# terran-project/terran

Measured on AMD Instinct MI355X. Metric: frames/sec 1080p detect+embed+pose, higher is better.
Workload: dtype f16x3: operands x = hi + lo (two IEEE halfs, 22 bits), 3 f16 MFMAs per product, f32 accumulate; float32-grade results; 1 GPU; BASELINE configs[4]: 1080p detect+embed+pose; Detection(short_side=416) + Recognition(top-2) + Estimation(short_side=184); 32 frames per GPU per step resident in HBM; random-init weights; precision=f16x3, frames_per_gpu_step=32, faces_per_frame=2, resident_batch_reused=True, batches_in_flight_per_gpu=2

## Files before the change

include/terran_amd.h:

```cpp
#ifndef TERRAN_AMD_H
#define TERRAN_AMD_H

#include <stddef.h>
#include <stdint.h>

#ifdef __cplusplus
extern "C" {
#endif

#define TA_OK 0
#define TA_E_INVALID (-1)
#define TA_E_DEVICE (-2)
#define TA_E_CAPACITY (-3)
#define TA_E_OVERFLOW (-4)
#define TA_E_RANGE (-5)

#define TA_MODEL_RETINAFACE 1
#define TA_MODEL_ARCFACE 2
#define TA_MODEL_OPENPOSE 3

typedef struct ta_ctx ta_ctx;
typedef struct ta_model ta_model;
typedef struct ta_frames ta_frames;

// ... 109 lines not shown
int ta_jpeg_encode_last_opt_stats(const ta_ctx* ctx, double* ms);

int ta_model_load(ta_ctx* ctx, int kind, const void* blob, size_t bytes, ta_model** out);
int ta_program_check(int kind, const void* blob, size_t bytes, char* msg, size_t msg_capacity);
void ta_model_free(ta_model* m);
int ta_model_kind(const ta_model* m);

int ta_model_forward_frames(ta_model* m, const ta_frames* frames);
int ta_model_forward_crops(ta_model* m, const uint8_t* crops_nchw_bgr, int n);
int ta_model_tensor_shape(ta_model* m, int tensor, int* n, int* c, int* h, int* w);
int ta_model_read_tensor(ta_model* m, int tensor, int ch_off, int ch, float* dst_nchw);

int ta_model_tensor_unscale(const ta_model* m, int tensor, float* out, int capacity);
int ta_model_debug_amax(ta_model* m, int enable, float* out, int capacity);
int ta_model_graph_probe(ta_model* m, int reps, double* out_ms);

int ta_retinaface_run(ta_model* m, const ta_frames* frames, float score_thr, float nms_thr,
                      int capacity, int32_t* counts, float* boxes, float* landmarks, float* scores,
                      int32_t* required);
int ta_retinaface_postprocess(ta_ctx* ctx, const float* const heads[9], int n, int h, int w,
                              float score_thr, float nms_thr, int capacity, int32_t* counts,
                              float* boxes, float* landmarks, float* scores, int32_t* required);

int ta_arcface_embed_crops(ta_model* m, const uint8_t* crops_nchw_bgr, int n, int normalize, float* out);
int ta_arcface_embed_faces(ta_model* m, const ta_frames* frames, const int32_t* frame_index,
                           const double* inv_affine, int n, int normalize, float* out,
                           uint8_t* crops_out);
int ta_arcface_embed_faces_multi(ta_model* m, const ta_frames* const* frames, int n_sources, const int32_t* source_index,
                                 const int32_t* frame_index, const double* inv_affine, int n, int normalize,
                                 float* out, uint8_t* crops_out);
int ta_cosine_distance(ta_ctx* ctx, const float* a, int na, const float* b, int nb, int dim, float* out);

int ta_openpose_run(ta_model* m, const ta_frames* frames, double scale, int capacity,
                    int32_t* counts, int32_t* keypoints, double* scores, int32_t* required);
int ta_openpose_group(ta_ctx* ctx, const float* pafs, const float* heatmaps, int n, int h, int w,
                      double scale, int capacity, int32_t* counts, int32_t* keypoints,
                      double* scores, int32_t* required);
int ta_openpose_last_stats(const ta_ctx* ctx, int64_t* peaks, int64_t* connections);

int ta_openpose_debug_read(ta_ctx* ctx, int n, int cap_peaks, int32_t* peak_counts, int32_t* peaks_yx,
                           float* peak_scores, int cap_conn, int32_t* conn_counts, int32_t* conn_ij,
                           float* conn_scores);

int ta_bicubic_x8(ta_ctx* ctx, const float* maps, int n, int c, int h, int w, float* out);

#define TA_CONV_AUTO 0
// ... 22 lines not shown
```

terran_amd/csrc/conv_dwpw.hip:

```cpp
#include <stdlib.h>

#include "conv_common.h"

TA_TRACE_READER(ta_debug_trace_read_dwpw)

template <int WAVES_M, int WAVES_N, int WM_TILES, int WN_TILES, int PREC = PREC_F32>
__global__ __launch_bounds__(256, 2) void conv_dwpw(const ta_conv_launch p) {
  constexpr int BN = WAVES_M * WM_TILES * 32;
  constexpr int BM = WAVES_N * WN_TILES * 32;
  constexpr int QA = BN / 32;
  constexpr int RP = BM / 32;
  constexpr int STAGE = (BN + BM) * 32;
  static_assert(WAVES_M * WAVES_N == 4, "4 waves per workgroup");
  extern __shared__ __attribute__((aligned(16))) float lds[];

  const int tid = threadIdx.x;
  const int lane = tid & 63;
  const int wave = __builtin_amdgcn_readfirstlane(tid >> 6);
  const int wm = wave / WAVES_N;
  const int wn = wave % WAVES_N;
  const int n_ct = p.coutp / BN;
  const int bid = blockIdx.x;
  const int grp = bid >> 3, xcd = bid & 7;
  const int ct = grp % n_ct;
// ... 84 lines not shown
  const int b_row0 = BN + wn * WN_TILES * 32 + frow;

  const int S = p.n_slabs;
  if (wave == 0) TA_STAMP(17);
  produce(0, 0);
  if (wave == 0) TA_STAMP(18);
  for (int s = 0; s < S; ++s) {
    asm volatile("s_waitcnt vmcnt(0)" ::: "memory");
    __syncthreads();
    if (s == 0 && wave == 0) TA_STAMP(19);
    if (s + 1 < S) produce(s + 1, (s + 1) & 1);
    const float* st = lds + (s & 1) * STAGE;
    conv_slab_mma<WM_TILES, WN_TILES, PREC>(st, acc, a_row0, b_row0, fsw, fcb, lane);
  }
  if (wave == 0) TA_STAMP(20);
  if constexpr (PREC != PREC_F32) {
    if (dw_amax > TA_F16_MAX_BITS) *p.range_flag = 1;
    if (p.amax_index >= 0 && dw_amax) atomicMax((unsigned*)p.range_flag + TA_AMAX_SLOT0 + 2 * p.amax_index + 1, dw_amax);
  }
  conv_finish_sym<WAVES_M, WAVES_N, WM_TILES, WN_TILES>(p, acc, lds, ct0, pt0, wm, wn, tid, lane, HoWo);
  if (wave == 0) TA_STAMP(23);
}

template <int WAVES_M, int WAVES_N, int WM_TILES, int WN_TILES>
__global__ __launch_bounds__(256, 2) void rf_dwpw_kernel(const ta_conv_launch p) {
  constexpr int BN = WAVES_M * WM_TILES * 32, BM = WAVES_N * WN_TILES * 32;
  constexpr int QA = BN / 32, RP = BM / 32, STAGE = (BN + BM) * 32;
  static_assert(WAVES_M * WAVES_N == 4 && (RP == 2 || RP == 4), "4 waves; 64 or 128 pixels per tile");
  extern __shared__ __attribute__((aligned(16))) float lds[];
  const int tid = threadIdx.x;
  const int lane = tid & 63;
  const int wave = __builtin_amdgcn_readfirstlane(tid >> 6);
  const int wm = wave / WAVES_N, wn = wave % WAVES_N;
  const int n_ct = p.coutp / BN;
  const int bid = blockIdx.x;
  const int grp = bid >> 3, xcd = bid & 7;
  const int ct = grp % n_ct;
  const int n_pt = (p.M + BM - 1) / BM;
  const int pt = ta_xcd_tile(n_pt, xcd, grp / n_ct);
  if (pt < 0) return;
  const int ct0 = ct * BN, pt0 = pt * BM;
  const int HoWo = p.Ho * p.Wo;
  const int C = p.dw_c, S = p.n_slabs;

  f32x4 pre[4];
  {
    const int pco = ct0 + 8 * (tid % (BN / 8));
// ... 29 lines not shown
      const int t = q * 4 + wave;
      __builtin_amdgcn_global_load_lds(GLB_PTR(a_src[q] + (size_t)s * a_slab_bytes), LDS_PTR(base + t * 256), 16, 0, 0);
    }
  };

  const int c4 = tid & 7;
  const __amdgpu_buffer_rsrc_t rsrc = __builtin_amdgcn_make_buffer_rsrc((void*)p.in, 0, -1, 0x00020000);
  int voff[RP];
#pragma unroll
  for (int j = 0; j < RP; ++j) {
    const int row = (tid >> 3) + 32 * j;
    int pix = pt0 + row;
    if (pix >= p.M) pix = 0;
    const int img = pix / HoWo;
    const int rem = pix - img * HoWo;
    const int y = rem / p.Wo;
    const int x = rem - y * p.Wo;
    voff[j] = 4 * (img * p.in_img + y * p.dw_stride * p.in_row + x * p.dw_stride * p.in_pix + p.in_off0) + 16 * c4;
  }
  const int row_b = 4 * p.in_row, pix_b = 4 * p.in_pix;

  unsigned dw_amax = 0;
  typedef unsigned u32x4 __attribute__((ext_vector_type(4)));
  auto produce = [&](int s, int stage) {
    float* base = lds + stage * STAGE;
    const int ch = s * 32 + c4 * 4;
    f32x4 w9[9], bias;
#pragma unroll
    for (int t = 0; t < 9; ++t) w9[t] = *(const f32x4*)(wl + t * C + ch);
    bias = *(const f32x4*)(wl + 9 * C + ch);
#pragma unroll
    for (int j0 = 0; j0 < RP; j0 += 2) {
      f32x4 v[2][9];
#pragma unroll
      for (int jj = 0; jj < 2; ++jj)
#pragma unroll
        for (int ky = 0; ky < 3; ++ky)
#pragma unroll
          for (int kx = 0; kx < 3; ++kx)
            v[jj][ky * 3 + kx] = __builtin_bit_cast(f32x4, (u32x4)__builtin_amdgcn_raw_buffer_load_b128(rsrc, voff[j0 + jj], ky * row_b + kx * pix_b + s * 128, 0));
#pragma unroll
      for (int jj = 0; jj < 2; ++jj) {
        const int row = (tid >> 3) + 32 * (j0 + jj);
        f32x4 acc = bias;
#pragma unroll
        for (int t = 0; t < 9; ++t)
#pragma unroll
          for (int e = 0; e < 4; ++e) acc[e] = __builtin_fmaf(v[jj][t][e], w9[t][e], acc[e]);
#pragma unroll
        for (int e = 0; e < 4; ++e) acc[e] = ta_relu(acc[e]);
        dw_amax = ta_amax4(dw_amax, acc);
        unsigned h0, h1, l0, l1;
        ta_pack2<true>(acc[0], acc[1], h0, l0);
        ta_pack2<true>(acc[2], acc[3], h1, l1);
        const int sw = (row >> 1) & 7;
        float* r = base + (BN + row) * 32 + (c4 & 1) * 2;
        *(uint2*)(r + (((c4 >> 1)) ^ sw) * 4) = make_uint2(h0, h1);
        *(uint2*)(r + ((4 + (c4 >> 1)) ^ sw) * 4) = make_uint2(l0, l1);
      }
    }
  };

  f32x16 acc[WM_TILES][WN_TILES];
// ... 19 lines not shown
        al[a] = *(const bf16x8*)(st + (a_row0 + a * 32) * 32 + ((4 + 2 * kg + t) ^ fsw) * 4);
      }
#pragma unroll
      for (int b = 0; b < WN_TILES; ++b) {
        bh[b] = *(const bf16x8*)(st + (b_row0 + b * 32) * 32 + ((2 * kg + t) ^ fsw) * 4);
        bl[b] = *(const bf16x8*)(st + (b_row0 + b * 32) * 32 + ((4 + 2 * kg + t) ^ fsw) * 4);
      }
#pragma unroll
      for (int a = 0; a < WM_TILES; ++a)
#pragma unroll
        for (int b = 0; b < WN_TILES; ++b) acc[a][b] = ta_mfma16<PREC_F16X3>(al[a], bh[b], acc[a][b]);
#pragma unroll
      for (int a = 0; a < WM_TILES; ++a)
#pragma unroll
        for (int b = 0; b < WN_TILES; ++b) acc[a][b] = ta_mfma16<PREC_F16X3>(ah[a], bl[b], acc[a][b]);
#pragma unroll
      for (int a = 0; a < WM_TILES; ++a)
#pragma unroll
        for (int b = 0; b < WN_TILES; ++b) acc[a][b] = ta_mfma16<PREC_F16X3>(ah[a], bh[b], acc[a][b]);
    }
  };

  dma_w(0, 0);
#pragma unroll
  for (int i = 0; i < WG; ++i)
    if (tid + 256 * i < n_gran) *(f32x4*)(wl + (tid + 256 * i) * 4) = wtmp[i];
  for (int g = tid + 256 * WG; g < n_gran; g += 256)
    *(f32x4*)(wl + g * 4) = g * 4 < 9 * C ? *(const f32x4*)(p.dw_w + g * 4) : *(const f32x4*)(p.dw_bias + (g * 4 - 9 * C));
  __syncthreads();
  produce(0, 0);
  for (int s = 0; s < S; ++s) {
    asm volatile("s_waitcnt vmcnt(0) lgkmcnt(0)" ::: "memory");
    __syncthreads();
    if (s + 1 < S) {
      dma_w(s + 1, (s + 1) & 1);
      produce(s + 1, (s + 1) & 1);
    }
    mma(s);
  }
  if (dw_amax > TA_F16_MAX_BITS) *p.range_flag = 1;
  if (p.amax_index >= 0 && dw_amax) atomicMax((unsigned*)p.range_flag + TA_AMAX_SLOT0 + 2 * p.amax_index + 1, dw_amax);

  constexpr int NCH = BN / 4, G = BN / 8, RPI = 256 / G;
  __syncthreads();
#pragma unroll
  for (int b = 0; b < WN_TILES; ++b) {
    const int row = (wn * WN_TILES + b) * 32 + (lane & 31);
#pragma unroll
    for (int a = 0; a < WM_TILES; ++a)
#pragma unroll
      for (int j = 0; j < 4; ++j) {
        const int c = ((wm * WM_TILES + a) * 32 + 8 * j + 4 * (lane >> 5)) >> 2;
        *(f32x4*)(lds + (row * NCH + (c ^ (row & (NCH - 1)))) * 4) =
            f32x4{acc[a][b][4 * j], acc[a][b][4 * j + 1], acc[a][b][4 * j + 2], acc[a][b][4 * j + 3]};
      }
  }
  __syncthreads();
  const int k8 = tid % G, r0 = tid / G;
  const int co = ct0 + 8 * k8;
// ... 24 lines not shown
        ta_split_store8<1>(o, v, am);
        amax = max(amax, am);
      } else {
        *(f32x4*)o = *(const f32x4*)v;
        *(f32x4*)(o + 16) = *(const f32x4*)(v + 4);
        if (chk) {
#pragma unroll
          for (int e = 0; e < 8; ++e) amax = max(amax, ta_absbits(v[e]));
        }
      }
      x += RPI;
      while (x >= p.Wo) {
        x -= p.Wo;
        if (++y == p.Ho) {
          y = 0;
          ++img;
        }
      }
    }
  }
  ta_range_report(p, amax);
}

template <int WAVES_M, int WAVES_N, int WM_TILES, int WN_TILES>
static int launch_rf_dwpw(ta_ctx* ctx, const ta_conv_launch& p) {
  constexpr int BN = WAVES_M * WM_TILES * 32, BM = WAVES_N * WN_TILES * 32;
  const int groups = ta_tile_grid(p, BN, BM).groups;
  const size_t lds_bytes = 2 * (size_t)(BN + BM) * 32 * sizeof(float) + (size_t)40 * p.dw_c;
  auto kern = rf_dwpw_kernel<WAVES_M, WAVES_N, WM_TILES, WN_TILES>;
  TA_NOTE_KERNEL(ctx, "rf_dwpw_kernel<%d,%d,%d,%d>", WAVES_M, WAVES_N, WM_TILES, WN_TILES);
  TA_SET_LDS_ATTR(ctx, kern, lds_bytes);
  hipLaunchKernelGGL(kern, dim3(groups * 8), dim3(256), lds_bytes, ctx->stream, p);
  TA_HIP(ctx, hipGetLastError());
  return TA_OK;
}

template <int WAVES_M, int WAVES_N, int WM_TILES, int WN_TILES, int PREC>
static int launch_dwpw_cfg(ta_ctx* ctx, const ta_conv_launch& p) {
  constexpr int BN = WAVES_M * WM_TILES * 32;
  constexpr int BM = WAVES_N * WN_TILES * 32;
  const int groups = ta_tile_grid(p, BN, BM).groups;
  const size_t lds_bytes = 2 * (size_t)(BN + BM) * 32 * sizeof(float);
  auto kern = conv_dwpw<WAVES_M, WAVES_N, WM_TILES, WN_TILES, PREC>;
  TA_NOTE_KERNEL(ctx, "conv_dwpw<%d,%d,%d,%d,%d>", WAVES_M, WAVES_N, WM_TILES, WN_TILES, PREC);
  TA_SET_LDS_ATTR(ctx, kern, lds_bytes);
  hipLaunchKernelGGL(kern, dim3(groups * 8), dim3(256), lds_bytes, ctx->stream, p);
  TA_HIP(ctx, hipGetLastError());
  return TA_OK;
}

int ta_launch_dwpw(ta_ctx* ctx, const ta_conv_launch& p_in, double flops) {
  if (p_in.M <= 0) return TA_OK;
  ta_conv_launch p = p_in;
  p.range_flag = ctx->range_flag;
  if ((p.prec != PREC_F32 && p.prec != PREC_F16X3) || p.in_fmt != TA_FMT_F32 || p.coutp % 32 || p.cout % 4 || (p.out_ch & 7) || p.dw_c % 4 || !p.dw_w ||
      !p.dw_bias || p.n_slabs * 32 < p.dw_c)
    return ta_fail(ctx, TA_E_INVALID, "dw+pw: needs the f32 or f16x3 mode, float32 input activations and 4-aligned channels");
  ta_prof_scope scope(ctx, 0, flops);
  ctx->cur_flops = flops;
#ifdef TA_CONV_TRACE
  p.trace_block = ctx->conv_trace_block;
#endif
  if (p.prec == PREC_F16X3) {
    const bool generic_only = getenv("TA_DWPW_GENERIC") != nullptr;
    const bool lean_ok = !generic_only && p.dw_c % 32 == 0 && p.dw_c == p.n_slabs * 32 && p.dw_c <= 1024 && p.cout % 8 == 0 && p.act == TA_ACT_RELU &&
                         (p.out_fmt == TA_FMT_F32 || p.out_fmt == TA_FMT_SPLIT16);
    if (lean_ok) {
      if (p.coutp % 128 == 0) return launch_rf_dwpw<2, 2, 2, 1>(ctx, p);
      if (p.coutp % 64 == 0) return launch_rf_dwpw<2, 2, 1, 1>(ctx, p);
      return launch_rf_dwpw<1, 4, 1, 1>(ctx, p);
    }
    if (p.coutp % 128 == 0) return launch_dwpw_cfg<2, 2, 2, 2, PREC_F16X3>(ctx, p);
    if (p.coutp % 64 == 0) return launch_dwpw_cfg<1, 4, 2, 1, PREC_F16X3>(ctx, p);
    return launch_dwpw_cfg<1, 4, 1, 1, PREC_F16X3>(ctx, p);
  }
  if (p.coutp % 128 == 0) return launch_dwpw_cfg<2, 2, 2, 2, PREC_F32>(ctx, p);
  if (p.coutp % 64 == 0) return launch_dwpw_cfg<1, 4, 2, 1, PREC_F32>(ctx, p);
  return launch_dwpw_cfg<1, 4, 1, 1, PREC_F32>(ctx, p);
}
```

terran_amd/csrc/retinaface_post.hip:

```cpp
#include <string.h>
#include <vector>

#include "act_format.h"
#include "ta_internal.h"

typedef float f32x4 __attribute__((ext_vector_type(4)));
#define RF_THREADS 1024
#define RF_LDS_KEYS 8192
#define RF_FAST_C 1024
#define RF_FAST_LDS (24 * 1024 + (RF_FAST_C / 64) * (RF_FAST_C / 64 + 1) / 2 * 64 * 8)
#define RF_LDS_MAX (159 * 1024)

struct rf_level {
  const float* head;
  int img, row, pix, off0;
  int fh, fw, stride;
  int t0;
  float ref[2][4];
};

struct rf_params {
  rf_level lv[3];
  int T;
  int cls_is_prob;
  float score_thr, nms_thr;
  float margin;
  unsigned long long* keys;
  int p_max;
  float* boxes;
  float* lmks;
  float* scores;
  int* keep;
  int* counts;
  int* ncand;
  long long* dbg;
  int fast_max;
};

__device__ __forceinline__ const float* rf_cell(const rf_level& L, int img, int t, int& a) {
  const int cell = t >> 1;
  a = t & 1;
  const int y = cell / L.fw, x = cell - y * L.fw;
  return L.head + (size_t)img * L.img + (size_t)y * L.row + (size_t)x * L.pix + L.off0;
}

__device__ __forceinline__ float rf_score(const rf_params& p, int img, int t) {
  const int l = t >= p.lv[2].t0 ? 2 : (t >= p.lv[1].t0 ? 1 : 0);
  int a;
  const float* c = rf_cell(p.lv[l], img, t - p.lv[l].t0, a);
  if (p.cls_is_prob) return c[2 + a];
  const float bg = c[a], fg = c[2 + a];
  const float m = fmaxf(bg, fg);
  const float eb = expf(bg - m), ef = expf(fg - m);
  return ef / (eb + ef);
}

__device__ __forceinline__ unsigned long long rf_readlane64(unsigned long long v, int l) {
  const unsigned lo = (unsigned)__builtin_amdgcn_readlane((int)(unsigned)v, l);
  const unsigned hi = (unsigned)__builtin_amdgcn_readlane((int)(unsigned)(v >> 32), l);
  return ((unsigned long long)hi << 32) | lo;
}

__device__ __forceinline__ int rf_row_off(int i, int W) {
  const int b = i >> 6;
  return 64 * (b * W - b * (b - 1) / 2) + (i - 64 * b) * (W - b);
}

__global__ __launch_bounds__(RF_THREADS) void rf_select_kernel(const rf_params p) {
  extern __shared__ __attribute__((aligned(16))) unsigned char smem[];
  unsigned long long* lkeys = (unsigned long long*)smem;
  unsigned* flags = (unsigned*)(smem + (size_t)RF_LDS_KEYS * 8);
  int* wave_tot = (int*)(flags + ((p.T + 31) / 32 + 3) / 4 * 4);
  int& s_base = wave_tot[16];

  const int img = blockIdx.x;
  const int tid = threadIdx.x, lane = tid & 63, wv = tid >> 6;
  unsigned long long* gkeys = p.keys + (size_t)img * p.p_max;

  if (p.dbg && tid == 0) p.dbg[img * 8 + 0] = wall_clock64();
  const int ncell = p.T >> 1;
  const int perc = (ncell + RF_THREADS - 1) / RF_THREADS;
  const int c0 = tid * perc, c1 = (c0 + perc < ncell) ? c0 + perc : ncell;
  const int per = 2 * perc, a0 = 2 * c0, a1 = 2 * c1;
  int cnt = 0;
  unsigned long long bits = 0;
  if (c0 < c1) {
    int l = a0 >= p.lv[2].t0 ? 2 : (a0 >= p.lv[1].t0 ? 1 : 0);
    const int cell = (a0 - p.lv[l].t0) >> 1;
    int y = cell / p.lv[l].fw, x = cell - y * p.lv[l].fw;
    const float* c = p.lv[l].head + (size_t)img * p.lv[l].img + (size_t)y * p.lv[l].row + (size_t)x * p.lv[l].pix + p.lv[l].off0;
    for (int q = c0; q < c1; q += 4) {
      f32x4 v[4];
#pragma unroll
      for (int k = 0; k < 4; ++k) {
        v[k] = *(const f32x4*)c;
        if (q + k + 1 < c1) {
          c += p.lv[l].pix;
          if (++x == p.lv[l].fw) {
            x = 0;
            ++y;
            c = p.lv[l].head + (size_t)img * p.lv[l].img + (size_t)y * p.lv[l].row + p.lv[l].off0;
          }
          if (l < 2 && 2 * (q + k + 1) == p.lv[l + 1].t0) {
            ++l;
            x = y = 0;
            c = p.lv[l].head + (size_t)img * p.lv[l].img + p.lv[l].off0;
          }
        }
// ... 3 lines not shown
#pragma unroll
        for (int a = 0; a < 2; ++a) {
          if (q + k >= c1) continue;
          bool pass;
          if (p.cls_is_prob) {
            pass = v[k][2 + a] >= p.score_thr;
          } else {
            const float bg = v[k][a], fg = v[k][2 + a];
            pass = false;
            if (!(fg - bg < p.margin)) {
              const float m = fmaxf(bg, fg);
              const float eb = expf(bg - m), ef = expf(fg - m);
              pass = ef / (eb + ef) >= p.score_thr;
            }
          }
          if (pass) {
            ++cnt;
            const int o = 2 * (q + k - c0) + a;
            if (o < 64) bits |= 1ull << o;
          }
        }
    }
  }
  int incl = cnt;
#pragma unroll
  for (int d = 1; d < 64; d <<= 1) {
    const int o = __shfl_up(incl, d, 64);
    if (lane >= d) incl += o;
  }
  if (lane == 63) wave_tot[wv] = incl;
  __syncthreads();
  int off = incl - cnt;
  for (int w = 0; w < wv; ++w) off += wave_tot[w];
  if (tid == RF_THREADS - 1) s_base = off + cnt;
  if (per <= 64) {
    while (bits) {
      const int t = a0 + __builtin_ctzll(bits);
      bits &= bits - 1;
      const unsigned hi = 0xFFFFFFFFu - __float_as_uint(rf_score(p, img, t));
      gkeys[off++] = ((unsigned long long)hi << 32) | (unsigned)t;
    }
  } else {
    for (int t = a0; t < a1; ++t) {
      const float sc = rf_score(p, img, t);
      if (sc >= p.score_thr) gkeys[off++] = ((unsigned long long)(0xFFFFFFFFu - __float_as_uint(sc)) << 32) | (unsigned)t;
    }
  }
  __syncthreads();
  const int C = s_base;
  if (tid == 0) p.ncand[img] = C;
  if (C == 0) {
    if (tid == 0) p.counts[img] = 0;
    return;
  }

  if (p.dbg && tid == 0) p.dbg[img * 8 + 1] = wall_clock64();
  int P = 1;
  while (P < C) P <<= 1;
  unsigned long long* keys = (P <= RF_LDS_KEYS) ? lkeys : gkeys;
  for (int i = tid; i < P; i += RF_THREADS) {
    const unsigned long long k = i < C ? gkeys[i] : ~0ull;
    if (keys != gkeys || i >= C) keys[i] = k;
  }
  __syncthreads();
  for (int k = 2; k <= P; k <<= 1) {
    for (int j = k >> 1; j > 0; j >>= 1) {
      for (int i = tid; i < P; i += RF_THREADS) {
        const int ixj = i ^ j;
        if (ixj > i) {
          const unsigned long long a = keys[i], b = keys[ixj];
          const bool up = (i & k) == 0;
          if ((a > b) == up) {
            keys[i] = b;
            keys[ixj] = a;
          }
        }
      }
      __syncthreads();
    }
  }

  if (p.dbg && tid == 0) p.dbg[img * 8 + 2] = wall_clock64();
  const bool fast = C <= p.fast_max && keys == lkeys;
  f32x4* sbox = (f32x4*)(smem + 8 * 1024);
  unsigned long long* smask = (unsigned long long*)(smem + 24 * 1024);
// ... 111 lines not shown
}

__global__ __launch_bounds__(256) void rf_gather_kernel(const rf_params p, int N, float* o_boxes, float* o_lmks,
                                                         float* o_scores) {
  const int img = blockIdx.x;
  int base = 0;
  for (int i = 0; i < img; ++i) base += p.counts[i];
  const int K = p.counts[img];
  const int* keep = p.keep + (size_t)img * p.T;
  const float* boxes = p.boxes + (size_t)img * p.T * 4;
  const float* lmks = p.lmks + (size_t)img * p.T * 10;
  const float* scores = p.scores + (size_t)img * p.T;
  for (int k = threadIdx.x; k < K; k += blockDim.x) {
    const int i = keep[k];
    const int o = base + k;
#pragma unroll
    for (int e = 0; e < 4; ++e) o_boxes[o * 4 + e] = boxes[i * 4 + e];
#pragma unroll
    for (int e = 0; e < 10; ++e) o_lmks[o * 10 + e] = lmks[i * 10 + e];
    o_scores[o] = scores[i];
  }
}

static void anchor_refs(int stride, float ref[2][4]) {
  const int scales[3][2] = {{32, 16}, {8, 4}, {2, 1}};
  const int li = stride == 32 ? 0 : (stride == 16 ? 1 : 2);
  const float ctr = 0.5f * (16 - 1);
  for (int a = 0; a < 2; ++a) {
    const float half = 0.5f * (16.0f * scales[li][a] - 1.0f);
    ref[a][0] = ctr - half;
    ref[a][1] = ctr - half;
    ref[a][2] = ctr + half;
    ref[a][3] = ctr + half;
  }
}

static int rf_postprocess_dev(ta_ctx* ctx, const ta_tensor heads[3], int N, int H, int W, int cls_is_prob,
                              float score_thr, float nms_thr, int capacity, int32_t* counts, float* boxes,
                              float* landmarks, float* scores, int32_t* required) {
  if (N <= 0) {
    if (required) *required = 0;
    return TA_OK;
  }
  rf_params p;
  memset(&p, 0, sizeof(p));
  const int strides[3] = {32, 16, 8};
// ... 16 lines not shown
    T += fh * fw * 2;
  }
  p.T = T;
  p.cls_is_prob = cls_is_prob;
  p.score_thr = score_thr;
  p.margin = -INFINITY;
  if (score_thr > 1e-4f && score_thr < 1.0f - 1e-4f) {
    const double lg = log((double)score_thr / (1.0 - (double)score_thr));
    p.margin = (float)(lg - 0.01 - 0.001 * fabs(lg));
  }
  p.nms_thr = nms_thr;
  int pmax = 1;
  while (pmax < T) pmax <<= 1;
  p.p_max = pmax;
  size_t off = 0;
  auto carve = [&](size_t bytes) {
    size_t o = off;
    off += (bytes + 255) & ~(size_t)255;
    return o;
  };
  const size_t o_keys = carve((size_t)N * pmax * 8), o_boxes = carve((size_t)N * T * 16), o_lmks = carve((size_t)N * T * 40);
  const size_t o_scores = carve((size_t)N * T * 4), o_keep = carve((size_t)N * T * 4), o_counts = carve((size_t)N * 4);
  const size_t o_ncand = carve((size_t)N * 4);
  const size_t cap = capacity > 0 ? (size_t)capacity : 0;
  const size_t o_ob = carve(cap * 16), o_ol = carve(cap * 40), o_os = carve(cap * 4);
  char* scr = nullptr;
  TA_TRY(ta_scratch(ctx, off, (void**)&scr));
  p.keys = (unsigned long long*)(scr + o_keys);
  p.boxes = (float*)(scr + o_boxes);
  p.lmks = (float*)(scr + o_lmks);
  p.scores = (float*)(scr + o_scores);
  p.keep = (int*)(scr + o_keep);
  p.counts = (int*)(scr + o_counts);
  p.ncand = (int*)(scr + o_ncand);
  size_t lds = (size_t)RF_LDS_KEYS * 8 + (size_t)(((T + 31) / 32 + 3) / 4 * 4) * 4 + 32 * 4;
  if (lds < RF_FAST_LDS) lds = RF_FAST_LDS;
  if (lds > RF_LDS_MAX) return ta_fail(ctx, TA_E_OVERFLOW, "retinaface: %d anchors per image exceed the NMS bitmap limit", T);
  static long long* dbg_dev = nullptr;
  if (getenv("TA_RF_DEBUG") && !dbg_dev) (void)hipMalloc((void**)&dbg_dev, 8 * 8 * 4096);
  p.dbg = dbg_dev;
  static const int fast_max = getenv("TA_RF_FAST_MAX") ? atoi(getenv("TA_RF_FAST_MAX")) : RF_FAST_C;
  p.fast_max = fast_max < RF_FAST_C ? fast_max : RF_FAST_C;
  {
    ta_prof_scope scope(ctx, 3, (double)N * T * 32 * 4);
    TA_SET_LDS_ATTR(ctx, rf_select_kernel, RF_LDS_MAX);
    hipLaunchKernelGGL(rf_select_kernel, dim3(N), dim3(RF_THREADS), lds, ctx->stream, p);
    TA_HIP(ctx, hipGetLastError());
  }
  TA_HIP(ctx, hipMemcpyAsync(counts, p.counts, (size_t)N * 4, hipMemcpyDeviceToHost, ctx->stream));
  TA_HIP(ctx, hipStreamSynchronize(ctx->stream));
  if (dbg_dev) {
    std::vector<long long> h(8 * N);
    (void)hipMemcpy(h.data(), dbg_dev, 8 * 8 * N, hipMemcpyDeviceToHost);
    for (int i = 0; i < N; ++i) fprintf(stderr, "rf img %d C %lld kept %lld: compact %.1f sort %.1f decode %.1f matrix %.1f scan %.1f us\n", i, h[8*i+6], h[8*i+7], (h[8*i+1]-h[8*i])/100.0, (h[8*i+2]-h[8*i+1])/100.0, (h[8*i+3]-h[8*i+2])/100.0, (h[8*i+4]-h[8*i+3])/100.0, (h[8*i+5]-h[8*i+4])/100.0);
  }
  long long total = 0;
  for (int i = 0; i < N; ++i) total += counts[i];
  if (required) *required = (int32_t)total;
  if (total > capacity) return ta_fail(ctx, TA_E_CAPACITY, "retinaface: %lld detections, capacity %d", total, capacity);
  if (total == 0) return TA_OK;
  hipLaunchKernelGGL(rf_gather_kernel, dim3(N), dim3(256), 0, ctx->stream, p, N, (float*)(scr + o_ob), (float*)(scr + o_ol),
                     (float*)(scr + o_os));
  TA_HIP(ctx, hipGetLastError());
  TA_HIP(ctx, hipMemcpyAsync(boxes, scr + o_ob, (size_t)total * 16, hipMemcpyDeviceToHost, ctx->stream));
  TA_HIP(ctx, hipMemcpyAsync(landmarks, scr + o_ol, (size_t)total * 40, hipMemcpyDeviceToHost, ctx->stream));
  TA_HIP(ctx, hipMemcpyAsync(scores, scr + o_os, (size_t)total * 4, hipMemcpyDeviceToHost, ctx->stream));
  TA_HIP(ctx, hipStreamSynchronize(ctx->stream));
  return TA_OK;
}

extern "C" {

int ta_retinaface_run(ta_model* m, const ta_frames* frames, float score_thr, float nms_thr, int capacity,
                      int32_t* counts, float* boxes, float* landmarks, float* scores, int32_t* required) {
  ta_enter(m ? m->ctx : nullptr);
  if (!m || !frames || !counts) return TA_E_INVALID;
  ta_ctx* ctx = m->ctx;
  if (m->kind != TA_MODEL_RETINAFACE) return ta_fail(ctx, TA_E_INVALID, "retinaface_run: wrong model kind");
  if (capacity > 0 && (!boxes || !landmarks || !scores)) return ta_fail(ctx, TA_E_INVALID, "retinaface_run: null outputs");
  if (frames->n == 0) {
    if (required) *required = 0;
    return TA_OK;
  }
  TA_TRY(ta_model_forward_frames(m, frames));
  TA_TRY(ta_range_enqueue(ctx));
  ta_tensor heads[3];
  for (int l = 0; l < 3; ++l) {
    heads[l] = m->tensor(m->hdr.outputs[l]);
    if (heads[l].unscale_dev || heads[l].fmt != TA_FMT_F32) return ta_fail(ctx, TA_E_INVALID, "retinaface_run: the head tensors must be plain float32");
  }
  const int rc = rf_postprocess_dev(ctx, heads, frames->n, frames->h, frames->w, 0, score_thr, nms_thr, capacity, counts, boxes,
                                    landmarks, scores, required);
  return ta_range_finish(ctx, rc);
}
// ... 55 lines not shown
```

terran_amd/csrc/runtime.hip:

```cpp
#include <stdarg.h>
#include <stdlib.h>
#include <string.h>

#include "ta_internal.h"

int ta_fail(ta_ctx* ctx, int code, const char* fmt, ...) {
  char buf[1024];
  va_list ap;
  va_start(ap, fmt);
  vsnprintf(buf, sizeof(buf), fmt, ap);
  va_end(ap);
  if (ctx) ctx->err = buf;
  return code;
}

int ta_scratch(ta_ctx* ctx, size_t bytes, void** out) {
  if (bytes > ctx->scratch_bytes) {
    TA_HIP(ctx, hipStreamSynchronize(ctx->stream));
    if (ctx->scratch) (void)hipFree(ctx->scratch);
    ctx->scratch = nullptr;
    ctx->scratch_bytes = 0;
    size_t want = bytes + bytes / 4 + (1 << 20);
    TA_HIP(ctx, hipMalloc(&ctx->scratch, want));
    ctx->scratch_bytes = want;
// ... 112 lines not shown
    const char* spin = getenv("TERRAN_AMD_SPIN_WAIT");
    if (!(spin && spin[0] && spin[0] != '0')) {
      (void)hipSetDeviceFlags(hipDeviceScheduleBlockingSync);
      (void)hipGetLastError();
    }
  }
  ta_ctx* ctx = new ta_ctx();
  ctx->device = device_id;
  if (hipStreamCreateWithFlags(&ctx->stream, hipStreamNonBlocking) != hipSuccess) {
    delete ctx;
    return TA_E_DEVICE;
  }
  (void)hipEventCreate(&ctx->t0);
  (void)hipEventCreate(&ctx->t1);
  const size_t flag_bytes = sizeof(int) * (TA_AMAX_SLOT0 + 2 * TA_AMAX_OPS);
  if (hipMalloc((void**)&ctx->range_flag, flag_bytes) != hipSuccess || hipMemset(ctx->range_flag, 0, flag_bytes) != hipSuccess ||
      hipHostMalloc((void**)&ctx->range_flag_host, sizeof(int), hipHostMallocDefault) != hipSuccess) {
    if (ctx->range_flag) (void)hipFree(ctx->range_flag);
    (void)hipStreamDestroy(ctx->stream);
    delete ctx;
    return TA_E_DEVICE;
  }
  *ctx->range_flag_host = 0;
  if (const char* e = getenv("TA_CONV_PREFER")) ctx->conv_force = atoi(e);
#ifdef TA_CONV_TRACE
  if (const char* e = getenv("TA_CONV_TRACE_BLOCK")) ctx->conv_trace_block = atoi(e);
#endif
  *out = ctx;
  return TA_OK;
}

void ta_ctx_destroy(ta_ctx* ctx) {
  if (!ctx) return;
  (void)hipSetDevice(ctx->device);
  (void)hipStreamSynchronize(ctx->stream);
  ta_drain_profile(ctx);
  for (auto e : ctx->event_pool) (void)hipEventDestroy(e);
  if (ctx->t0) (void)hipEventDestroy(ctx->t0);
  if (ctx->t1) (void)hipEventDestroy(ctx->t1);
  if (ctx->scratch) (void)hipFree(ctx->scratch);
  if (ctx->pinned) (void)hipHostFree(ctx->pinned);
  if (ctx->pose_wphase) (void)hipFree(ctx->pose_wphase);
  if (ctx->jpeg_enc_dev) (void)hipFree(ctx->jpeg_enc_dev);
  if (ctx->jpeg_enc_out) (void)hipHostFree(ctx->jpeg_enc_out);
  ta_pose_free_big(ctx);
  if (ctx->range_flag) (void)hipFree(ctx->range_flag);
// ... 424 lines not shown
```

terran_amd/csrc/ta_internal.h:

```cpp
#pragma once
#include <hip/hip_runtime.h>
#include <stdint.h>
#include <stdio.h>
#include <atomic>
#include <map>
#include <memory>
#include <mutex>
#include <string>
#include <vector>

#include "../../include/terran_amd.h"

#define TA_BLOB_MAGIC 0x314D4154u

enum {
  TA_OP_CONV = 1,
  TA_OP_DWCONV = 2,
  TA_OP_MAXPOOL = 3,
  TA_OP_COPYCH = 4,
  TA_OP_RFSTEM = 5,
  TA_OP_DWPW = 6
};
enum { TA_ACT_NONE = 0, TA_ACT_RELU = 1, TA_ACT_PRELU = 2 };

// ... 80 lines not shown
  double jpeg_enc_ms[8] = {0, 0, 0, 0, 0, 0, 0, 0};
  int64_t jpeg_enc_counts[4] = {0, 0, 0, 0};
  double jpeg_enc_opt_ms[2] = {0, 0};
  void* jpeg_enc_dev = nullptr;
  size_t jpeg_enc_dev_bytes = 0;
  uint8_t* jpeg_enc_out = nullptr;
  size_t jpeg_enc_out_bytes = 0;
  float* pose_wphase = nullptr;
  struct {
    int n = 0, maxp = 0;
    const int *peak_cnt = nullptr, *peak_yx = nullptr, *conn_cnt = nullptr, *conn_ij = nullptr;
    const float *peak_sc = nullptr, *conn_sc = nullptr;
    struct over_t {
      int img, maxp;
      void* mem;
      const int *peak_cnt, *peak_yx, *conn_cnt, *conn_ij;
      const float *peak_sc, *conn_sc;
    };
    std::vector<over_t> over;
  } pose_dbg;
  hipStream_t side_stream[2] = {nullptr, nullptr};
  hipEvent_t side_fork[2] = {nullptr, nullptr}, side_join[2] = {nullptr, nullptr};
  int conv_force = 0;
#ifdef TA_CONV_TRACE
  int conv_trace_block = 0;
#endif
  int64_t conv_counts[16] = {0};
  int* range_flag = nullptr;
  int* range_flag_host = nullptr;
  const void* amax_owner = nullptr;
  double cur_flops = 0;
  std::map<std::string, std::pair<int64_t, double>> kernel_work;
  std::map<std::string, double> kernel_ms;
  const std::string* cur_kernel = nullptr;
  void note_kernel(const char* name) {
    auto it = kernel_work.try_emplace(name, 0, 0.0).first;
    it->second.first += 1;
    it->second.second += cur_flops;
    cur_kernel = &it->first;
  }
};
void ta_pose_free_big(ta_ctx* ctx);
#define TA_AMAX_SLOT0 16
#define TA_AMAX_OPS 4096
int ta_range_enqueue(ta_ctx* ctx);
int ta_range_check(ta_ctx* ctx);
// ... 231 lines not shown
```

terran_amd/lib.py:

```python
import ctypes as C
import os

import numpy as np

HERE = os.path.dirname(os.path.abspath(__file__))
LIB_PATH = os.path.join(HERE, 'libterran_amd.so')

OK, E_INVALID, E_DEVICE, E_CAPACITY, E_OVERFLOW, E_RANGE = 0, -1, -2, -3, -4, -5
_CODES = {E_INVALID: 'TA_E_INVALID', E_DEVICE: 'TA_E_DEVICE', E_CAPACITY: 'TA_E_CAPACITY', E_OVERFLOW: 'TA_E_OVERFLOW',
          E_RANGE: 'TA_E_RANGE'}


class TerranAmdError(RuntimeError):
    def __init__(self, code, msg):
        super().__init__('%s: %s' % (_CODES.get(code, code), msg))
        self.code = code


c_int, c_float, c_double, c_void_p, c_size_t = C.c_int, C.c_float, C.c_double, C.c_void_p, C.c_size_t
P = C.POINTER
u8p, i32p, f32p, f64p = P(C.c_uint8), P(C.c_int32), P(C.c_float), P(C.c_double)

SIGNATURES = {
    'ta_version': (C.c_char_p, []),
# ... 30 lines not shown
                               P(C.c_int32)]),
    'ta_jpeg_last_stats': (c_int, [c_void_p, c_void_p, c_void_p]),
    'ta_jpeg_encode_header': (c_int, [c_int, c_int, c_int, c_int, c_void_p, c_size_t, P(c_size_t)]),
    'ta_jpeg_encode': (c_int, [c_void_p, c_void_p, c_int, c_int, P(c_void_p), P(c_size_t)]),
    'ta_jpeg_encode_last_stats': (c_int, [c_void_p, c_void_p, c_void_p]),
    'ta_jpeg_encode_opt': (c_int, [c_void_p, c_void_p, c_int, c_int, c_int, P(c_void_p), P(c_size_t)]),
    'ta_jpeg_optimal_table': (c_int, [c_void_p, c_void_p, c_void_p, P(c_int)]),
    'ta_jpeg_encode_last_opt_stats': (c_int, [c_void_p, c_void_p]),
    'ta_program_check': (c_int, [c_int, c_void_p, c_size_t, C.c_char_p, c_size_t]),
    'ta_model_load': (c_int, [c_void_p, c_int, c_void_p, c_size_t, P(c_void_p)]),
    'ta_model_free': (None, [c_void_p]),
    'ta_model_kind': (c_int, [c_void_p]),
    'ta_model_forward_frames': (c_int, [c_void_p, c_void_p]),
    'ta_model_forward_crops': (c_int, [c_void_p, c_void_p, c_int]),
    'ta_model_tensor_shape': (c_int, [c_void_p, c_int, P(c_int), P(c_int), P(c_int), P(c_int)]),
    'ta_model_tensor_unscale': (c_int, [c_void_p, c_int, c_void_p, c_int]),
    'ta_model_debug_amax': (c_int, [c_void_p, c_int, c_void_p, c_int]),
    'ta_model_graph_probe': (c_int, [c_void_p, c_int, c_void_p]),
    'ta_model_read_tensor': (c_int, [c_void_p, c_int, c_int, c_int, c_void_p]),
    'ta_retinaface_run': (c_int, [c_void_p, c_void_p, c_float, c_float, c_int, c_void_p, c_void_p, c_void_p,
                                  c_void_p, P(C.c_int32)]),
    'ta_retinaface_postprocess': (c_int, [c_void_p, P(c_void_p), c_int, c_int, c_int, c_float, c_float, c_int,
                                          c_void_p, c_void_p, c_void_p, c_void_p, P(C.c_int32)]),
    'ta_arcface_embed_crops': (c_int, [c_void_p, c_void_p, c_int, c_int, c_void_p]),
    'ta_arcface_embed_faces': (c_int, [c_void_p, c_void_p, c_void_p, c_void_p, c_int, c_int, c_void_p, c_void_p]),
    'ta_arcface_embed_faces_multi': (c_int, [c_void_p, P(c_void_p), c_int, c_void_p, c_void_p, c_void_p, c_int, c_int, c_void_p,
                                             c_void_p]),
    'ta_cosine_distance': (c_int, [c_void_p, c_void_p, c_int, c_void_p, c_int, c_int, c_void_p]),
    'ta_openpose_run': (c_int, [c_void_p, c_void_p, c_double, c_int, c_void_p, c_void_p, c_void_p, P(C.c_int32)]),
    'ta_openpose_group': (c_int, [c_void_p, c_void_p, c_void_p, c_int, c_int, c_int, c_double, c_int, c_void_p,
                                  c_void_p, c_void_p, P(C.c_int32)]),
    'ta_bicubic_x8': (c_int, [c_void_p, c_void_p, c_int, c_int, c_int, c_int, c_void_p]),
    'ta_openpose_last_stats': (c_int, [c_void_p, c_void_p, c_void_p]),
    'ta_openpose_debug_read': (c_int, [c_void_p, c_int, c_int, c_void_p, c_void_p, c_void_p, c_int, c_void_p, c_void_p,
                                       c_void_p]),
    'ta_debug_conv_variant': (c_int, [c_void_p, c_int]),
    'ta_debug_range_check': (c_int, [c_void_p]),
    'ta_debug_conv_counts': (c_int, [c_void_p, c_void_p, c_int]),
    'ta_debug_kernel_work': (c_int, [c_void_p, C.c_char_p, c_size_t, c_int]),
}

DRAW_BAR, DRAW_LINE, DRAW_DISC, DRAW_MASK = 0, 1, 2, 3
PRIM_DT = np.dtype([('frame', '<i4'), ('kind', '<i4'), ('x0', '<i4'), ('y0', '<i4'), ('x1', '<i4'), ('y1', '<i4'),
                    ('width', '<i4'), ('rgba', 'u1', (4,))])
assert PRIM_DT.itemsize == 32

# ... 499 lines not shown
```

Baseline: 2210 frames/s.

## Split RetinaFace candidate scoring across segments and prefetch dwpw first-stage taps

RetinaFace candidate selection used one workgroup per image to scan every anchor. A new score kernel now spreads that scan over up to 31 segment workgroups per image, each writing its candidates to a segment buffer. The select kernel then prefix-sums the segment counts and gathers the candidates before sorting and NMS. Separately, the depthwise+pointwise lean kernel issues the first slab's 3x3 tap loads before the weight LDS fill, to hide load latency in the prologue. A 32-bit offset bound check is also added to the lean path. This costs an extra launch, more scratch memory and extra registers.

Result: no change. 2205 frames/s (median of 2 runs) (-0.2%).

```diff
diff --git a/include/terran_amd.h b/include/terran_amd.h
--- a/include/terran_amd.h
+++ b/include/terran_amd.h
@@ -155,6 +155,9 @@
                               float score_thr, float nms_thr, int capacity, int32_t* counts,
                               float* boxes, float* landmarks, float* scores, int32_t* required);
 
+int ta_retinaface_segments(int h, int w, int32_t* seg_cells, int32_t* segments);
+int ta_debug_dwpw_kernel(const int32_t* fields, int n);
+
 int ta_arcface_embed_crops(ta_model* m, const uint8_t* crops_nchw_bgr, int n, int normalize, float* out);
 int ta_arcface_embed_faces(ta_model* m, const ta_frames* frames, const int32_t* frame_index,
                            const double* inv_affine, int n, int normalize, float* out,
diff --git a/terran_amd/csrc/conv_dwpw.hip b/terran_amd/csrc/conv_dwpw.hip
--- a/terran_amd/csrc/conv_dwpw.hip
+++ b/terran_amd/csrc/conv_dwpw.hip
@@ -1,4 +1,5 @@
 #include <stdlib.h>
+#include <string.h>
 
 #include "conv_common.h"
 
@@ -130,7 +131,7 @@
   if (wave == 0) TA_STAMP(23);
 }
 
-template <int WAVES_M, int WAVES_N, int WM_TILES, int WN_TILES>
+template <int WAVES_M, int WAVES_N, int WM_TILES, int WN_TILES, bool PRO>
 __global__ __launch_bounds__(256, 2) void rf_dwpw_kernel(const ta_conv_launch p) {
   constexpr int BN = WAVES_M * WM_TILES * 32, BM = WAVES_N * WN_TILES * 32;
   constexpr int QA = BN / 32, RP = BM / 32, STAGE = (BN + BM) * 32;
@@ -206,7 +207,17 @@
 
   unsigned dw_amax = 0;
   typedef unsigned u32x4 __attribute__((ext_vector_type(4)));
-  auto produce = [&](int s, int stage) {
+  auto taps = [&](int s, int j0, f32x4 (*v)[9]) {
+#pragma unroll
+    for (int jj = 0; jj < 2; ++jj)
+#pragma unroll
+      for (int ky = 0; ky < 3; ++ky)
+#pragma unroll
+        for (int kx = 0; kx < 3; ++kx)
+          v[jj][ky * 3 + kx] = __builtin_bit_cast(f32x4, (u32x4)__builtin_amdgcn_raw_buffer_load_b128(rsrc, voff[j0 + jj], ky * row_b + kx * pix_b + s * 128, 0));
+  };
+  f32x4 v0[2][9];
+  auto produce = [&](int s, int stage, bool have0) {
     float* base = lds + stage * STAGE;
     const int ch = s * 32 + c4 * 4;
     f32x4 w9[9], bias;
@@ -216,13 +227,14 @@
 #pragma unroll
     for (int j0 = 0; j0 < RP; j0 += 2) {
       f32x4 v[2][9];
-#pragma unroll
-      for (int jj = 0; jj < 2; ++jj)
-#pragma unroll
-        for (int ky = 0; ky < 3; ++ky)
-#pragma unroll
-          for (int kx = 0; kx < 3; ++kx)
-            v[jj][ky * 3 + kx] = __builtin_bit_cast(f32x4, (u32x4)__builtin_amdgcn_raw_buffer_load_b128(rsrc, voff[j0 + jj], ky * row_b + kx * pix_b + s * 128, 0));
+      if (have0 && j0 == 0) {
+#pragma unroll
+        for (int jj = 0; jj < 2; ++jj)
+#pragma unroll
+          for (int t = 0; t < 9; ++t) v[jj][t] = v0[jj][t];
+      } else {
+        taps(s, j0, v);
+      }
 #pragma unroll
       for (int jj = 0; jj < 2; ++jj) {
         const int row = (tid >> 3) + 32 * (j0 + jj);
@@ -288,19 +300,20 @@
   };
 
   dma_w(0, 0);
+  if constexpr (PRO) taps(0, 0, v0);
 #pragma unroll
   for (int i = 0; i < WG; ++i)
     if (tid + 256 * i < n_gran) *(f32x4*)(wl + (tid + 256 * i) * 4) = wtmp[i];
   for (int g = tid + 256 * WG; g < n_gran; g += 256)
     *(f32x4*)(wl + g * 4) = g * 4 < 9 * C ? *(const f32x4*)(p.dw_w + g * 4) : *(const f32x4*)(p.dw_bias + (g * 4 - 9 * C));
   __syncthreads();
-  produce(0, 0);
+  produce(0, 0, PRO);
   for (int s = 0; s < S; ++s) {
     asm volatile("s_waitcnt vmcnt(0) lgkmcnt(0)" ::: "memory");
     __syncthreads();
     if (s + 1 < S) {
       dma_w(s + 1, (s + 1) & 1);
-      produce(s + 1, (s + 1) & 1);
+      produce(s + 1, (s + 1) & 1, false);
     }
     mma(s);
   }
@@ -371,17 +384,23 @@
   ta_range_report(p, amax);
 }
 
-template <int WAVES_M, int WAVES_N, int WM_TILES, int WN_TILES>
-static int launch_rf_dwpw(ta_ctx* ctx, const ta_conv_launch& p) {
+template <int WAVES_M, int WAVES_N, int WM_TILES, int WN_TILES, bool PRO>
+static int launch_rf_dwpw_pro(ta_ctx* ctx, const ta_conv_launch& p) {
   constexpr int BN = WAVES_M * WM_TILES * 32, BM = WAVES_N * WN_TILES * 32;
   const int groups = ta_tile_grid(p, BN, BM).groups;
   const size_t lds_bytes = 2 * (size_t)(BN + BM) * 32 * sizeof(float) + (size_t)40 * p.dw_c;
-  auto kern = rf_dwpw_kernel<WAVES_M, WAVES_N, WM_TILES, WN_TILES>;
+  auto kern = rf_dwpw_kernel<WAVES_M, WAVES_N, WM_TILES, WN_TILES, PRO>;
   TA_NOTE_KERNEL(ctx, "rf_dwpw_kernel<%d,%d,%d,%d>", WAVES_M, WAVES_N, WM_TILES, WN_TILES);
   TA_SET_LDS_ATTR(ctx, kern, lds_bytes);
   hipLaunchKernelGGL(kern, dim3(groups * 8), dim3(256), lds_bytes, ctx->stream, p);
   TA_HIP(ctx, hipGetLastError());
   return TA_OK;
+}
+
+template <int WAVES_M, int WAVES_N, int WM_TILES, int WN_TILES>
+static int launch_rf_dwpw(ta_ctx* ctx, const ta_conv_launch& p) {
+  return ctx->dwpw_prologue && p.dw_c >= 128 ? launch_rf_dwpw_pro<WAVES_M, WAVES_N, WM_TILES, WN_TILES, true>(ctx, p)
+                            : launch_rf_dwpw_pro<WAVES_M, WAVES_N, WM_TILES, WN_TILES, false>(ctx, p);
 }
 
 template <int WAVES_M, int WAVES_N, int WM_TILES, int WN_TILES, int PREC>
@@ -396,6 +415,17 @@
   hipLaunchKernelGGL(kern, dim3(groups * 8), dim3(256), lds_bytes, ctx->stream, p);
   TA_HIP(ctx, hipGetLastError());
   return TA_OK;
+}
+
+static bool ta_dwpw_lean_ok(const ta_conv_launch& p) {
+  if (!(p.dw_c % 32 == 0 && p.dw_c == p.n_slabs * 32 && p.dw_c <= 1024 && p.cout % 8 == 0 && p.act == TA_ACT_RELU &&
+        (p.out_fmt == TA_FMT_F32 || p.out_fmt == TA_FMT_SPLIT16)))
+    return false;
+  const long long HoWo = (long long)p.Ho * p.Wo;
+  const long long n_img = HoWo > 0 ? (p.M + HoWo - 1) / HoWo : 0;
+  const long long in_end = ((n_img + 1) * p.in_img + p.in_off0 + 2ll * p.in_row + 2ll * p.in_pix) * 4;
+  const long long out_end = ((n_img + 1) * p.out_img + p.out_off0) * 4;
+  return in_end < (1ll << 32) && out_end < (1ll << 32);
 }
 
 int ta_launch_dwpw(ta_ctx* ctx, const ta_conv_launch& p_in, double flops) {
@@ -412,8 +442,7 @@
 #endif
   if (p.prec == PREC_F16X3) {
     const bool generic_only = getenv("TA_DWPW_GENERIC") != nullptr;
-    const bool lean_ok = !generic_only && p.dw_c % 32 == 0 && p.dw_c == p.n_slabs * 32 && p.dw_c <= 1024 && p.cout % 8 == 0 && p.act == TA_ACT_RELU &&
-                         (p.out_fmt == TA_FMT_F32 || p.out_fmt == TA_FMT_SPLIT16);
+    const bool lean_ok = !generic_only && ta_dwpw_lean_ok(p);
     if (lean_ok) {
       if (p.coutp % 128 == 0) return launch_rf_dwpw<2, 2, 2, 1>(ctx, p);
       if (p.coutp % 64 == 0) return launch_rf_dwpw<2, 2, 1, 1>(ctx, p);
@@ -427,3 +456,13 @@
   if (p.coutp % 64 == 0) return launch_dwpw_cfg<1, 4, 2, 1, PREC_F32>(ctx, p);
   return launch_dwpw_cfg<1, 4, 1, 1, PREC_F32>(ctx, p);
 }
+
+extern "C" int ta_debug_dwpw_kernel(const int32_t* f, int n) {
+  if (!f || n != 16) return TA_E_INVALID;
+  ta_conv_launch p;
+  memset(&p, 0, sizeof(p));
+  p.M = f[0], p.Ho = f[1], p.Wo = f[2], p.dw_c = f[3], p.n_slabs = f[4], p.cout = f[5], p.act = f[6], p.out_fmt = f[7];
+  p.in_img = f[8], p.in_row = f[9], p.in_pix = f[10], p.in_off0 = f[11];
+  p.out_img = f[12], p.out_row = f[13], p.out_pix = f[14], p.out_off0 = f[15];
+  return ta_dwpw_lean_ok(p) ? 1 : 0;
+}
diff --git a/terran_amd/csrc/retinaface_post.hip b/terran_amd/csrc/retinaface_post.hip
--- a/terran_amd/csrc/retinaface_post.hip
+++ b/terran_amd/csrc/retinaface_post.hip
@@ -6,6 +6,8 @@
 
 typedef float f32x4 __attribute__((ext_vector_type(4)));
 #define RF_THREADS 1024
+#define RF_SCORE_THREADS 256
+#define RF_MAX_SEGS 31
 #define RF_LDS_KEYS 8192
 #define RF_FAST_C 1024
 #define RF_FAST_LDS (24 * 1024 + (RF_FAST_C / 64) * (RF_FAST_C / 64 + 1) / 2 * 64 * 8)
@@ -35,6 +37,10 @@
   int* ncand;
   long long* dbg;
   int fast_max;
+  int nseg;
+  int seg_cells;
+  unsigned long long* cand;
+  int* seg_count;
 };
 
 __device__ __forceinline__ const float* rf_cell(const rf_level& L, int img, int t, int& a) {
@@ -66,24 +72,8 @@
   return 64 * (b * W - b * (b - 1) / 2) + (i - 64 * b) * (W - b);
 }
 
-__global__ __launch_bounds__(RF_THREADS) void rf_select_kernel(const rf_params p) {
-  extern __shared__ __attribute__((aligned(16))) unsigned char smem[];
-  unsigned long long* lkeys = (unsigned long long*)smem;
-  unsigned* flags = (unsigned*)(smem + (size_t)RF_LDS_KEYS * 8);
-  int* wave_tot = (int*)(flags + ((p.T + 31) / 32 + 3) / 4 * 4);
-  int& s_base = wave_tot[16];
-
-  const int img = blockIdx.x;
-  const int tid = threadIdx.x, lane = tid & 63, wv = tid >> 6;
-  unsigned long long* gkeys = p.keys + (size_t)img * p.p_max;
-
-  if (p.dbg && tid == 0) p.dbg[img * 8 + 0] = wall_clock64();
-  const int ncell = p.T >> 1;
-  const int perc = (ncell + RF_THREADS - 1) / RF_THREADS;
-  const int c0 = tid * perc, c1 = (c0 + perc < ncell) ? c0 + perc : ncell;
-  const int per = 2 * perc, a0 = 2 * c0, a1 = 2 * c1;
-  int cnt = 0;
-  unsigned long long bits = 0;
+__device__ __forceinline__ void rf_scan_run(const rf_params& p, int img, int c0, int c1, int& cnt, unsigned long long& bits) {
+  const int a0 = 2 * c0;
   if (c0 < c1) {
     int l = a0 >= p.lv[2].t0 ? 2 : (a0 >= p.lv[1].t0 ? 1 : 0);
     const int cell = (a0 - p.lv[l].t0) >> 1;
@@ -133,6 +123,37 @@
         }
     }
   }
+}
+
+__device__ __forceinline__ void rf_emit_run(const rf_params& p, int img, int a0, int a1, unsigned long long bits,
+                                            unsigned long long* dst) {
+  if (a1 - a0 <= 64) {
+    while (bits) {
+      const int t = a0 + __builtin_ctzll(bits);
+      bits &= bits - 1;
+      const unsigned hi = 0xFFFFFFFFu - __float_as_uint(rf_score(p, img, t));
+      *dst++ = ((unsigned long long)hi << 32) | (unsigned)t;
+    }
+  } else {
+    for (int t = a0; t < a1; ++t) {
+      const float sc = rf_score(p, img, t);
+      if (sc >= p.score_thr) *dst++ = ((unsigned long long)(0xFFFFFFFFu - __float_as_uint(sc)) << 32) | (unsigned)t;
+    }
+  }
+}
+
+__global__ __launch_bounds__(RF_SCORE_THREADS) void rf_score_kernel(const rf_params p) {
+  __shared__ int wave_tot[RF_SCORE_THREADS / 64];
+  const int seg = blockIdx.x, img = blockIdx.y;
+  const int tid = threadIdx.x, lane = tid & 63, wv = tid >> 6;
+  const int ncell = p.T >> 1;
+  const int perc = p.seg_cells / RF_SCORE_THREADS;
+  int c0 = seg * p.seg_cells + tid * perc;
+  if (c0 > ncell) c0 = ncell;
+  const int c1 = (c0 + perc < ncell) ? c0 + perc : ncell;
+  int cnt = 0;
+  unsigned long long bits = 0;
+  rf_scan_run(p, img, c0, c1, cnt, bits);
   int incl = cnt;
 #pragma unroll
   for (int d = 1; d < 64; d <<= 1) {
@@ -143,35 +164,90 @@
   __syncthreads();
   int off = incl - cnt;
   for (int w = 0; w < wv; ++w) off += wave_tot[w];
-  if (tid == RF_THREADS - 1) s_base = off + cnt;
-  if (per <= 64) {
-    while (bits) {
-      const int t = a0 + __builtin_ctzll(bits);
-      bits &= bits - 1;
-      const unsigned hi = 0xFFFFFFFFu - __float_as_uint(rf_score(p, img, t));
-      gkeys[off++] = ((unsigned long long)hi << 32) | (unsigned)t;
-    }
+  const size_t sg = (size_t)img * p.nseg + seg;
+  if (tid == RF_SCORE_THREADS - 1) p.seg_count[sg] = off + cnt;
+  rf_emit_run(p, img, 2 * c0, 2 * c1, bits, p.cand + sg * (2 * (size_t)p.seg_cells) + off);
+}
+
+__global__ __launch_bounds__(RF_THREADS) void rf_select_kernel(const rf_params p) {
+  extern __shared__ __attribute__((aligned(16))) unsigned char smem[];
+  unsigned long long* lkeys = (unsigned long long*)smem;
+  unsigned* flags = (unsigned*)(smem + (size_t)RF_LDS_KEYS * 8);
+  int* wave_tot = (int*)(flags + ((p.T + 31) / 32 + 3) / 4 * 4);
+  int& s_base = wave_tot[16];
+
+  const int img = blockIdx.x;
+  const int tid = threadIdx.x, lane = tid & 63, wv = tid >> 6;
+  unsigned long long* gkeys = p.keys + (size_t)img * p.p_max;
+
+  if (p.dbg && tid == 0) p.dbg[img * 8 + 0] = wall_clock64();
+  int C, P = 1;
+  unsigned long long* keys;
+  if (p.nseg) {
+    int* seg_end = wave_tot;
+    if (wv == 0) {
+      int e = lane < p.nseg ? p.seg_count[(size_t)img * p.nseg + lane] : 0;
+#pragma unroll
+      for (int d = 1; d < 32; d <<= 1) {
+        const int o = __shfl_up(e, d, 64);
+        if (lane >= d) e += o;
+      }
+      if (lane < p.nseg) seg_end[lane] = e;
+    }
+    __syncthreads();
+    C = seg_end[p.nseg - 1];
+    if (tid == 0) p.ncand[img] = C;
+    if (C == 0) {
+      if (tid == 0) p.counts[img] = 0;
+      return;
+    }
+    if (p.dbg && tid == 0) p.dbg[img * 8 + 1] = wall_clock64();
+    while (P < C) P <<= 1;
+    keys = (P <= RF_LDS_KEYS) ? lkeys : gkeys;
+    const unsigned long long* cand = p.cand + (size_t)img * p.nseg * (2 * (size_t)p.seg_cells);
+    for (int i = tid; i < C; i += RF_THREADS) {
+      int lo = 0, hi = p.nseg - 1;
+      while (lo < hi) {
+        const int mid = (lo + hi) >> 1;
+        if (seg_end[mid] > i) hi = mid; else lo = mid + 1;
+      }
+      keys[i] = cand[(size_t)lo * (2 * (size_t)p.seg_cells) + (i - (lo ? seg_end[lo - 1] : 0))];
+    }
+    for (int i = C + tid; i < P; i += RF_THREADS) keys[i] = ~0ull;
   } else {
-    for (int t = a0; t < a1; ++t) {
-      const float sc = rf_score(p, img, t);
-      if (sc >= p.score_thr) gkeys[off++] = ((unsigned long long)(0xFFFFFFFFu - __float_as_uint(sc)) << 32) | (unsigned)t;
-    }
-  }
-  __syncthreads();
-  const int C = s_base;
-  if (tid == 0) p.ncand[img] = C;
-  if (C == 0) {
-    if (tid == 0) p.counts[img] = 0;
-    return;
-  }
-
-  if (p.dbg && tid == 0) p.dbg[img * 8 + 1] = wall_clock64();
-  int P = 1;
-  while (P < C) P <<= 1;
-  unsigned long long* keys = (P <= RF_LDS_KEYS) ? lkeys : gkeys;
-  for (int i = tid; i < P; i += RF_THREADS) {
-    const unsigned long long k = i < C ? gkeys[i] : ~0ull;
-    if (keys != gkeys || i >= C) keys[i] = k;
+    const int ncell = p.T >> 1;
+    const int perc = (ncell + RF_THREADS - 1) / RF_THREADS;
+    const int c0 = tid * perc, c1 = (c0 + perc < ncell) ? c0 + perc : ncell;
+    int cnt = 0;
+    unsigned long long bits = 0;
+    rf_scan_run(p, img, c0, c1, cnt, bits);
+    int incl = cnt;
+#pragma unroll
+    for (int d = 1; d < 64; d <<= 1) {
+      const int o = __shfl_up(incl, d, 64);
+      if (lane >= d) incl += o;
+    }
+    if (lane == 63) wave_tot[wv] = incl;
+    __syncthreads();
+    int off = incl - cnt;
+    for (int w = 0; w < wv; ++w) off += wave_tot[w];
+    if (tid == RF_THREADS - 1) s_base = off + cnt;
+    rf_emit_run(p, img, 2 * c0, 2 * c1, bits, gkeys + off);
+    __syncthreads();
+    C = s_base;
+    if (tid == 0) p.ncand[img] = C;
+    if (C == 0) {
+      if (tid == 0) p.counts[img] = 0;
+      return;
+    }
+
+    if (p.dbg && tid == 0) p.dbg[img * 8 + 1] = wall_clock64();
+    while (P < C) P <<= 1;
+    keys = (P <= RF_LDS_KEYS) ? lkeys : gkeys;
+    for (int i = tid; i < P; i += RF_THREADS) {
+      const unsigned long long k = i < C ? gkeys[i] : ~0ull;
+      if (keys != gkeys || i >= C) keys[i] = k;
+    }
   }
   __syncthreads();
   for (int k = 2; k <= P; k <<= 1) {
@@ -329,6 +405,13 @@
   }
 }
 
+static int rf_segments(int ncell, int* seg_cells) {
+  const int unit = RF_SCORE_THREADS * RF_MAX_SEGS;
+  const int perc = (ncell + unit - 1) / unit;
+  *seg_cells = RF_SCORE_THREADS * perc;
+  return (ncell + *seg_cells - 1) / *seg_cells;
+}
+
 static void anchor_refs(int stride, float ref[2][4]) {
   const int scales[3][2] = {{32, 16}, {8, 4}, {2, 1}};
   const int li = stride == 32 ? 0 : (stride == 16 ? 1 : 2);
@@ -391,6 +474,8 @@
   const size_t o_keys = carve((size_t)N * pmax * 8), o_boxes = carve((size_t)N * T * 16), o_lmks = carve((size_t)N * T * 40);
   const size_t o_scores = carve((size_t)N * T * 4), o_keep = carve((size_t)N * T * 4), o_counts = carve((size_t)N * 4);
   const size_t o_ncand = carve((size_t)N * 4);
+  if (ctx->rf_select_split) p.nseg = rf_segments(T / 2, &p.seg_cells);
+  const size_t o_cand = carve((size_t)N * p.nseg * 2 * p.seg_cells * 8), o_segc = carve((size_t)N * p.nseg * 4);
   const size_t cap = capacity > 0 ? (size_t)capacity : 0;
   const size_t o_ob = carve(cap * 16), o_ol = carve(cap * 40), o_os = carve(cap * 4);
   char* scr = nullptr;
@@ -402,6 +487,8 @@
   p.keep = (int*)(scr + o_keep);
   p.counts = (int*)(scr + o_counts);
   p.ncand = (int*)(scr + o_ncand);
+  p.cand = (unsigned long long*)(scr + o_cand);
+  p.seg_count = (int*)(scr + o_segc);
   size_t lds = (size_t)RF_LDS_KEYS * 8 + (size_t)(((T + 31) / 32 + 3) / 4 * 4) * 4 + 32 * 4;
   if (lds < RF_FAST_LDS) lds = RF_FAST_LDS;
   if (lds > RF_LDS_MAX) return ta_fail(ctx, TA_E_OVERFLOW, "retinaface: %d anchors per image exceed the NMS bitmap limit", T);
@@ -413,6 +500,11 @@
   {
     ta_prof_scope scope(ctx, 3, (double)N * T * 32 * 4);
     TA_SET_LDS_ATTR(ctx, rf_select_kernel, RF_LDS_MAX);
+    if (p.nseg) {
+      if (N > 65535) return ta_fail(ctx, TA_E_INVALID, "retinaface: more than 65535 images in one batch");
+      hipLaunchKernelGGL(rf_score_kernel, dim3(p.nseg, N), dim3(RF_SCORE_THREADS), 0, ctx->stream, p);
+      TA_HIP(ctx, hipGetLastError());
+    }
     hipLaunchKernelGGL(rf_select_kernel, dim3(N), dim3(RF_THREADS), lds, ctx->stream, p);
     TA_HIP(ctx, hipGetLastError());
   }
@@ -439,6 +531,16 @@
 }
 
 extern "C" {
+
+int ta_retinaface_segments(int h, int w, int32_t* seg_cells, int32_t* segments) {
+  if (h <= 0 || w <= 0 || !seg_cells || !segments) return TA_E_INVALID;
+  int ncell = 0;
+  for (int s = 32; s >= 8; s >>= 1) ncell += ((h + s - 1) / s) * ((w + s - 1) / s);
+  int sc = 0;
+  *segments = rf_segments(ncell, &sc);
+  *seg_cells = sc;
+  return TA_OK;
+}
 
 int ta_retinaface_run(ta_model* m, const ta_frames* frames, float score_thr, float nms_thr, int capacity,
                       int32_t* counts, float* boxes, float* landmarks, float* scores, int32_t* required) {
diff --git a/terran_amd/csrc/runtime.hip b/terran_amd/csrc/runtime.hip
--- a/terran_amd/csrc/runtime.hip
+++ b/terran_amd/csrc/runtime.hip
@@ -158,6 +158,8 @@
     return TA_E_DEVICE;
   }
   *ctx->range_flag_host = 0;
+  ctx->rf_select_split = getenv("TERRAN_AMD_NO_RF_SELECT_SPLIT") == nullptr;
+  ctx->dwpw_prologue = getenv("TERRAN_AMD_NO_DWPW_PROLOGUE") == nullptr;
   if (const char* e = getenv("TA_CONV_PREFER")) ctx->conv_force = atoi(e);
 #ifdef TA_CONV_TRACE
   if (const char* e = getenv("TA_CONV_TRACE_BLOCK")) ctx->conv_trace_block = atoi(e);
diff --git a/terran_amd/csrc/ta_internal.h b/terran_amd/csrc/ta_internal.h
--- a/terran_amd/csrc/ta_internal.h
+++ b/terran_amd/csrc/ta_internal.h
@@ -126,6 +126,8 @@
   hipStream_t side_stream[2] = {nullptr, nullptr};
   hipEvent_t side_fork[2] = {nullptr, nullptr}, side_join[2] = {nullptr, nullptr};
   int conv_force = 0;
+  bool rf_select_split = true;
+  bool dwpw_prologue = true;
 #ifdef TA_CONV_TRACE
   int conv_trace_block = 0;
 #endif
diff --git a/terran_amd/lib.py b/terran_amd/lib.py
--- a/terran_amd/lib.py
+++ b/terran_amd/lib.py
@@ -76,6 +76,8 @@
                                   c_void_p, P(C.c_int32)]),
     'ta_retinaface_postprocess': (c_int, [c_void_p, P(c_void_p), c_int, c_int, c_int, c_float, c_float, c_int,
                                           c_void_p, c_void_p, c_void_p, c_void_p, P(C.c_int32)]),
+    'ta_retinaface_segments': (c_int, [c_int, c_int, P(C.c_int32), P(C.c_int32)]),
+    'ta_debug_dwpw_kernel': (c_int, [c_void_p, c_int]),
     'ta_arcface_embed_crops': (c_int, [c_void_p, c_void_p, c_int, c_int, c_void_p]),
     'ta_arcface_embed_faces': (c_int, [c_void_p, c_void_p, c_void_p, c_void_p, c_int, c_int, c_void_p, c_void_p]),
     'ta_arcface_embed_faces_multi': (c_int, [c_void_p, P(c_void_p), c_int, c_void_p, c_void_p, c_void_p, c_int, c_int, c_void_p,
```
